# smallflyingpig/speech-to-image-translation-without-text

Measured on AMD Instinct MI355X. Metric: StackGAN-v2 3-stage G+D train-step images/sec at 256px, higher is better.
Workload: dtype f32

## Files before the change

include/s2i_hip.h:

```cpp
#ifndef S2I_HIP_H
#define S2I_HIP_H

#include <stddef.h>
#include <stdint.h>

#ifdef __cplusplus
extern "C" {
#endif

#define S2I_ABI_VERSION 4

#define S2I_CONV_K1      0
#define S2I_CONV_K3S1    1
#define S2I_CONV_K4S2    2
#define S2I_TCONV_K4S2   3

#define S2I_CONV_1D      4

#define S2I_ACT_NONE     0
#define S2I_ACT_GLU      1
#define S2I_ACT_LRELU    2
#define S2I_ACT_TANH     3
#define S2I_ACT_RELU     4

#define S2I_DT_F32       0
#define S2I_DT_BF16      1

#define S2I_PACK_PLAIN   0
#define S2I_PACK_UPFOLD  1

const char* s2i_last_error(void);
int  s2i_version(void);
int  s2i_set_tuning(const char* key, int value);
int  s2i_get_tuning(const char* key, int* value);
int  s2i_check_device(void);

typedef struct s2i_conv_desc {
  int kind;
  int B, H, W;
  int Cx;
  int Cc;
  int N;
  int wmode;
  int flip;
  int wR;
  int ldw;
  int act;
  int stats;
  int ldy;
  int groups;
  int nosplit;
  int kw, stride, pad;
  int tile_rows;
  int in_act;
  int in_groups;
} s2i_conv_desc;

size_t s2i_conv_workspace_bytes(const s2i_conv_desc* d);
int    s2i_conv_stat_parts(const s2i_conv_desc* d);
int s2i_conv_forward(const s2i_conv_desc* d, const float* x, const float* cvec, const float* w,
                     const float* bias, float* y, float* part, void* ws, size_t ws_bytes,
                     void* stream);

int s2i_conv_forward_cls(const s2i_conv_desc* d, const float* x, const float* cvec, const float* w,
                         const float* bias, const float* cls_bias, float* y, float* part, void* ws,
                         size_t ws_bytes, void* stream);

int s2i_conv_forward_in(const s2i_conv_desc* d, const float* x_raw, const float* in_coef, const float* w, float* y,
                        float* part, void* ws, size_t ws_bytes, void* stream);

int s2i_cvec_bias_table(const float* cvec, const float* packed, int B, int Cc, int Ip, int Op, int N,
                        float* table, void* ws , size_t ws_bytes, void* stream);
size_t s2i_border_sums_workspace_bytes(int B, int H, int W, int C);
int s2i_tap_sums(const float* dy, int B, int H, int W, int C, float* tapsum, void* ws, size_t ws_bytes,
                 void* stream);
int s2i_cvec_grads(const float* cvec, const float* packed, const float* tapsum, int B, int Cc, int Ip,
                   int Op, int N, int O, int I_total, float* dc, float* dw_oihw, int accumulate,
                   void* stream);

typedef struct s2i_wgrad_desc {
  int kind;
  int B, H, W;
  int Ca;
  int Cc;
  int N;
  int ldg;
  int swap;
  int fold;
  int O, I, KH, KW;
  int accumulate;
  int i_off;
  int I_total;
  int a_act;
  int a_groups;
} s2i_wgrad_desc;

size_t s2i_wgrad_workspace_bytes(const s2i_wgrad_desc* d);
int s2i_conv_wgrad(const s2i_wgrad_desc* d, const float* a, const float* cvec, const float* g,
                   float* grad_oihw, void* ws, size_t ws_bytes, void* stream);

int s2i_conv_wgrad_in_eligible(const s2i_wgrad_desc* d);
int s2i_conv_wgrad_in(const s2i_wgrad_desc* d, const float* a_raw, const float* a_coef, const float* g,
                      float* grad_oihw, void* ws, size_t ws_bytes, void* stream);


int s2i_conv_split_eligible(const s2i_conv_desc* d);
int s2i_conv_forward_split(const s2i_conv_desc* d, const float* x, const float* cvec,
                           const unsigned short* wsplit, int planes, int np, int kp, const float* bias,
                           const float* cls_bias, float* y, float* part, void* ws, size_t ws_bytes,
                           void* stream);
size_t s2i_wgrad_workspace_bytes_split(const s2i_wgrad_desc* d, int planes);
int s2i_conv_wgrad_split(const s2i_wgrad_desc* d, int planes, const float* a, const float* cvec,
                         const float* g, float* grad_oihw, void* ws, size_t ws_bytes, void* stream);
int s2i_split_packed_weight(const float* packed, int T, int R, int C, int planes, unsigned short* out_rc,
                            unsigned short* out_cr, void* stream);
// ... 243 lines not shown
```

speech_to_image_translation_without_text_amd/_lib.py:

```python
import ctypes
import os

import torch

_HERE = os.path.dirname(os.path.abspath(__file__))
LIB_PATH = os.path.join(_HERE, "libs2i_hip.so")

CONV_K1, CONV_K3S1, CONV_K4S2, TCONV_K4S2, CONV_1D = 0, 1, 2, 3, 4
ACT_NONE, ACT_GLU, ACT_LRELU, ACT_TANH, ACT_RELU = 0, 1, 2, 3, 4
PACK_PLAIN, PACK_UPFOLD = 0, 1
DT_F32, DT_BF16 = 0, 1
POOL_MAX3S2, POOL_AVG3S1, POOL_GLOBAL = 0, 1, 2
POOL_THEN_LRN, LRN_THEN_POOL = 0, 1
LOGMEL_BFT, LOGMEL_NHWC = 0, 1
ENC_LOSS_JEL, ENC_LOSS_L1, ENC_LOSS_DISTILL = 1, 2, 4
LOGMEL_TILE_FRAMES = 64
ABI_VERSION = 4

c_int, c_float, c_void_p, c_size_t, c_ll = (ctypes.c_int, ctypes.c_float, ctypes.c_void_p,
                                            ctypes.c_size_t, ctypes.c_longlong)


class ConvDesc(ctypes.Structure):
    _fields_ = [(n, c_int) for n in ("kind", "B", "H", "W", "Cx", "Cc", "N", "wmode", "flip", "wR",
                                     "ldw", "act", "stats", "ldy", "groups", "nosplit", "kw", "stride", "pad",
                                     "tile_rows", "in_act", "in_groups")]


class Conv2dDesc(ctypes.Structure):
    _fields_ = [(n, c_int) for n in ("B", "H", "W", "C", "ldx", "N", "kh", "kw", "sh", "sw", "ph", "pw", "Ho", "Wo",
                                     "ldy", "coff", "relu", "tile")]


class WgradDesc(ctypes.Structure):
    _fields_ = [(n, c_int) for n in ("kind", "B", "H", "W", "Ca", "Cc", "N", "ldg", "swap", "fold",
                                     "O", "I", "KH", "KW", "accumulate", "i_off", "I_total", "a_act", "a_groups")]


class PackItem(ctypes.Structure):
    _fields_ = [("w", c_void_p), ("packed", c_void_p)] + [(n, c_int) for n in ("O", "I", "KH", "KW", "Ip", "mode", "gx",
                                                                               "block0")]


class Pack16Item(ctypes.Structure):
    _fields_ = [("P", c_void_p), ("out", c_void_p)] + [(n, c_int) for n in (
        "R", "C", "kind", "flip", "transpose", "T", "nphase", "Nn", "Npad", "Kk", "CK", "gx", "gy", "block0")]


P = c_void_p
_SIGNATURES = {
    "s2i_last_error": (ctypes.c_char_p, []),
    "s2i_version": (c_int, []),
    "s2i_check_device": (c_int, []),
    "s2i_set_tuning": (c_int, [ctypes.c_char_p, c_int]),
    "s2i_get_tuning": (c_int, [ctypes.c_char_p, ctypes.POINTER(c_int)]),
    "s2i_conv_workspace_bytes": (c_size_t, [ctypes.POINTER(ConvDesc)]),
    "s2i_conv_stat_parts": (c_int, [ctypes.POINTER(ConvDesc)]),
    "s2i_conv_forward": (c_int, [ctypes.POINTER(ConvDesc), P, P, P, P, P, P, P, c_size_t, P]),
    "s2i_conv_forward_cls": (c_int, [ctypes.POINTER(ConvDesc), P, P, P, P, P, P, P, P, c_size_t, P]),
    "s2i_conv_forward_in": (c_int, [ctypes.POINTER(ConvDesc), P, P, P, P, P, P, c_size_t, P]),
    "s2i_conv_wgrad_in_eligible": (c_int, [ctypes.POINTER(WgradDesc)]),
    "s2i_conv_wgrad_in": (c_int, [ctypes.POINTER(WgradDesc), P, P, P, P, P, c_size_t, P]),
    "s2i_conv_split_eligible": (c_int, [ctypes.POINTER(ConvDesc)]),
    "s2i_conv_forward_split": (c_int, [ctypes.POINTER(ConvDesc), P, P, P, c_int, c_int, c_int, P, P, P, P, P, c_size_t, P]),
    "s2i_split_packed_weight": (c_int, [P, c_int, c_int, c_int, c_int, P, P, P]),
    "s2i_wgrad_workspace_bytes_split": (c_size_t, [ctypes.POINTER(WgradDesc), c_int]),
    "s2i_conv_wgrad_split": (c_int, [ctypes.POINTER(WgradDesc), c_int, P, P, P, P, P, c_size_t, P]),
    "s2i_conv_bf16_eligible": (c_int, [ctypes.POINTER(ConvDesc)]),
    "s2i_conv_bf16_workspace_bytes": (c_size_t, [ctypes.POINTER(ConvDesc)]),
    "s2i_conv_bf16_stat_parts": (c_int, [ctypes.POINTER(ConvDesc)]),
    "s2i_conv_bf16_weight_elems": (c_size_t, [ctypes.POINTER(ConvDesc)]),
    "s2i_conv_bf16_weight_layout": (c_int, [ctypes.POINTER(ConvDesc)]),
    "s2i_pack16_item_fill": (c_int, [ctypes.POINTER(ConvDesc), P, c_int, c_int, P, ctypes.POINTER(Pack16Item)]),
    "s2i_pack_conv_weights_bf16_batched": (c_int, [P, c_int, c_int, P]),
    "s2i_pack_conv_weight_bf16": (c_int, [ctypes.POINTER(ConvDesc), P, c_int, c_int, P, P]),
    "s2i_conv_forward_bf16": (c_int, [ctypes.POINTER(ConvDesc), P, P, P, P, P, P, c_size_t, P]),
    "s2i_conv_forward_dt": (c_int, [ctypes.POINTER(ConvDesc), P, c_int, P, P, P, P, P, c_int, P, P, c_size_t, P]),
    "s2i_wgrad_workspace_bytes_dt": (c_size_t, [ctypes.POINTER(WgradDesc), c_int, c_int]),
    "s2i_conv_wgrad_dt": (c_int, [ctypes.POINTER(WgradDesc), P, c_int, P, P, c_int, P, P, c_size_t, P]),
    "s2i_bn_act_forward_dt": (c_int, [c_int, P, c_ll, c_int, c_int, P, c_int, P, P, P]),
    "s2i_bn_act_bwd_reduce_dt": (c_int, [c_int, P, P, c_int, c_ll, c_int, c_int, P, c_int, P, c_int, P]),
    "s2i_bn_act_bwd_apply_dt": (c_int, [c_int, P, P, c_int, c_ll, c_int, c_int, P, P, c_int, P, P]),
    "s2i_act_backward_dt": (c_int, [c_int, P, P, c_int, c_ll, c_int, c_int, P, P]),
    "s2i_nchw_to_nhwc_dt": (c_int, [c_int, P, P, c_int, c_int, c_int, c_int, c_int, P]),
    "s2i_nhwc_to_nchw_dt": (c_int, [c_int, P, c_int, P, c_int, c_int, c_int, c_int, P]),
    "s2i_spatial_sum_dt": (c_int, [c_int, P, c_int, c_int, c_int, c_int, P, P, c_size_t, P]),
    "s2i_tap_sums_dt": (c_int, [c_int, P, c_int, c_int, c_int, c_int, P, P, c_size_t, P]),
    "s2i_cast": (c_int, [P, c_int, P, c_int, c_ll, P]),
    "s2i_cvec_bias_table": (c_int, [P, P, c_int, c_int, c_int, c_int, c_int, P, P, c_size_t, P]),
    "s2i_border_sums_workspace_bytes": (c_size_t, [c_int, c_int, c_int, c_int]),
    "s2i_tap_sums": (c_int, [P, c_int, c_int, c_int, c_int, P, P, c_size_t, P]),
    "s2i_cvec_grads": (c_int, [P, P, P, c_int, c_int, c_int, c_int, c_int, c_int, c_int, P, P, c_int, P]),
    "s2i_wgrad_workspace_bytes": (c_size_t, [ctypes.POINTER(WgradDesc)]),
    "s2i_conv_wgrad": (c_int, [ctypes.POINTER(WgradDesc), P, P, P, P, P, c_size_t, P]),
    "s2i_pack_conv_weight": (c_int, [P, P, c_int, c_int, c_int, c_int, c_int, c_int, P]),
    "s2i_pack_conv_weights_batched": (c_int, [P, c_int, c_int, c_int, P]),
    "s2i_bn_finalize": (c_int, [P, c_int, c_int, c_int, c_ll, P, P, P, P, P, c_float, c_float, P, P]),
    "s2i_bn_eval_coeffs": (c_int, [c_int, P, P, P, P, c_float, P, P]),
    "s2i_bn_act_forward": (c_int, [P, c_ll, c_int, c_int, P, c_int, P, P, P]),
    "s2i_colstats": (c_int, [P, c_ll, c_int, c_int, P, c_int, P]),
    "s2i_bn_act_bwd_reduce": (c_int, [P, P, c_int, c_ll, c_int, c_int, P, c_int, P, c_int, P]),
    "s2i_bn_bwd_finalize": (c_int, [P, c_int, c_int, c_int, c_ll, P, P, c_int, P, P]),
    "s2i_bn_act_bwd_apply": (c_int, [P, P, c_int, c_ll, c_int, c_int, P, P, c_int, P, P]),
    "s2i_act_backward": (c_int, [P, P, c_int, c_ll, c_int, c_int, P, P]),
    "s2i_glu_forward": (c_int, [P, c_ll, c_int, P, P]),
    "s2i_glu_backward": (c_int, [P, P, c_ll, c_int, P, P]),
    "s2i_nchw_to_nhwc": (c_int, [P, P, c_int, c_int, c_int, c_int, c_int, P]),
    "s2i_nhwc_to_nchw": (c_int, [P, c_int, P, c_int, c_int, c_int, c_int, P]),
# ... 152 lines not shown
```

speech_to_image_translation_without_text_amd/csrc/s2i_common.h:

```cpp
#pragma once
#include <hip/hip_runtime.h>
#include <stdio.h>
#include <stdarg.h>
#include "../../include/s2i_hip.h"

typedef float f32x16 __attribute__((ext_vector_type(16)));
typedef float f32x4 __attribute__((ext_vector_type(4)));

void s2i_set_error(const char* fmt, ...);

#define S2I_FAIL(...)            \
  do {                           \
    s2i_set_error(__VA_ARGS__);  \
    return 1;                    \
  } while (0)

#define S2I_REQUIRE(cond, ...)   \
  do {                           \
    if (!(cond)) S2I_FAIL(__VA_ARGS__); \
  } while (0)

#define S2I_LAUNCH_CHECK(name)                                          \
  do {                                                                  \
    hipError_t e__ = hipGetLastError();                                 \
    if (e__ != hipSuccess) S2I_FAIL("%s: launch failed: %s", name, hipGetErrorString(e__)); \
  } while (0)

static inline int s2i_ilog2(int v) {
  int l = 0;
  while ((1 << l) < v) ++l;
  return l;
}
static inline bool s2i_is_pow2(int v) { return v > 0 && (v & (v - 1)) == 0; }
static inline int s2i_cdiv(long long a, long long b) { return (int)((a + b - 1) / b); }

enum {
  S2I_TUNE_FWD_BM = 0,
  S2I_TUNE_FWD_MIN_CPS,
  S2I_TUNE_B16_V2,
  S2I_TUNE_B16_PERSIST,
  S2I_TUNE_FINALIZE_THREADS,
  S2I_TUNE_B16_DBG,
  S2I_TUNE_WGRAD16_BM,
  S2I_TUNE_WGRAD_BM,
  S2I_TUNE_COUNT
};
int s2i_tune(int key, int def);
```

speech_to_image_translation_without_text_amd/csrc/s2i_conv_fwd.hip:

```cpp
#include "s2i_igemm.h"

namespace {

template <int ASLOTS>
__device__ __forceinline__ void gather_rows(const IgemmP& p, int m0, int mrow, int kq, int s, int pad, int kw, int py, int px,
                                            int (&aoff)[ASLOTS], unsigned (&amask)[ASLOTS], int (&acoff)[ASLOTS]) {
#pragma unroll
  for (int i = 0; i < ASLOTS; ++i) {
    const int m = m0 + mrow + 32 * i;
    unsigned mask = 0;
    int base = 0, coff = 0;
    if (m < p.M) {
      int b, oy, ox;
      row_pixel(p, m, b, oy, ox);
      const int by = p.kind == S2I_CONV_1D ? oy : oy * s - pad, bx = ox * s - pad;
      mask = tap_mask(p.kind, kw, by, bx, p.H, p.W, py, px);
      base = (((b * p.H + by) * p.W + bx) * p.Cx + kq * 4) * 4;
      coff = (b * p.Cc + kq * 4) * 4;
    }
    aoff[i] = base;
    amask[i] = mask;
    acoff[i] = coff;
  }
}
// ... 541 lines not shown
    else if (act == S2I_ACT_TANH) v = tanhf(v);
    else if (act == S2I_ACT_RELU) v = fmaxf(v, 0.f);
    if (y16) reinterpret_cast<unsigned short*>(y)[row * ldy + n] = f2bf(v);
    else y[row * ldy + n] = v;
  }
}

__global__ __launch_bounds__(256) void splitk_reduce_stats_kernel(const float* __restrict__ slab, int S, long long rows,
                                                                  int N, float* __restrict__ y, int ldy,
                                                                  float* __restrict__ part, int nparts, int cpb,
                                                                  int ppg, long long Rg, int y16) {
  __shared__ f32x4 sh[2][256];
  const int tid = threadIdx.x;
  const int rpb = 256 / cpb;
  const int ql = tid % cpb, rl = tid / cpb;
  const int quad = blockIdx.y * cpb + ql;
  const int Q = N / 4;
  const int grp = blockIdx.x / ppg, pp = blockIdx.x - grp * ppg;
  const long long chunk = (Rg + ppg - 1) / ppg;
  const long long r0 = grp * Rg + pp * chunk;
  const long long gend = (grp + 1) * Rg < rows ? (grp + 1) * Rg : rows;
  const long long r1 = r0 + chunk < gend ? r0 + chunk : gend;
  const size_t sstride = (size_t)rows * N;
  f32x4 s0 = {0.f, 0.f, 0.f, 0.f}, s1 = {0.f, 0.f, 0.f, 0.f};
  if (quad < Q) {
    for (long long row = r0 + rl; row < r1; row += rpb) {
      const float* sp = slab + row * N + quad * 4;
      f32x4 v = *reinterpret_cast<const f32x4*>(sp);
      for (int s = 1; s < S; ++s) v += *reinterpret_cast<const f32x4*>(sp + s * sstride);
      if (y16) {
        unsigned short* yp = reinterpret_cast<unsigned short*>(y) + row * ldy + quad * 4;
        *reinterpret_cast<u32x2_t*>(yp) = u32x2_t{(unsigned)f2bf(v[0]) | ((unsigned)f2bf(v[1]) << 16),
                                                 (unsigned)f2bf(v[2]) | ((unsigned)f2bf(v[3]) << 16)};
      } else {
        *reinterpret_cast<f32x4*>(y + row * ldy + quad * 4) = v;
      }
      s0 += v;
      s1 += v * v;
    }
  }
  sh[0][tid] = s0;
  sh[1][tid] = s1;
  __syncthreads();
  if (rl == 0 && quad < Q) {
    for (int r = 1; r < rpb; ++r) {
      s0 += sh[0][r * cpb + ql];
      s1 += sh[1][r * cpb + ql];
    }
    *reinterpret_cast<f32x4*>(part + ((size_t)0 * nparts + blockIdx.x) * N + quad * 4) = s0;
    *reinterpret_cast<f32x4*>(part + ((size_t)1 * nparts + blockIdx.x) * N + quad * 4) = s1;
  }
}

template <int BM, int BN, int WM, int WN>
void launch_fwd(const IgemmP& p, dim3 grid, bool wt, bool ca32, hipStream_t st) {
  if (p.in_coef) {
    hipLaunchKernelGGL((igemm_fwd_kernel<BM, BN, WM, WN, false, true, true>), grid, dim3(256), 0, st, p);
    return;
  }
  if (wt) {
    if (ca32) hipLaunchKernelGGL((igemm_fwd_kernel<BM, BN, WM, WN, true, true>), grid, dim3(256), 0, st, p);
    else hipLaunchKernelGGL((igemm_fwd_kernel<BM, BN, WM, WN, true, false>), grid, dim3(256), 0, st, p);
  } else {
    if (ca32) hipLaunchKernelGGL((igemm_fwd_kernel<BM, BN, WM, WN, false, true>), grid, dim3(256), 0, st, p);
    else hipLaunchKernelGGL((igemm_fwd_kernel<BM, BN, WM, WN, false, false>), grid, dim3(256), 0, st, p);
  }
}

template <int BM, int BN, int WM, int WN>
static void launch_split(const IgemmP& p, dim3 grid, int planes, hipStream_t st) {
  if (planes == 1) hipLaunchKernelGGL((igemm_fwd_split_kernel<BM, BN, WM, WN, 1>), grid, dim3(256), 0, st, p);
  else if (planes == 2) hipLaunchKernelGGL((igemm_fwd_split_kernel<BM, BN, WM, WN, 2>), grid, dim3(256), 0, st, p);
  else hipLaunchKernelGGL((igemm_fwd_split_kernel<BM, BN, WM, WN, 3>), grid, dim3(256), 0, st, p);
}

}

int launch_igemm_fwd(const FwdPlan& pl, const IgemmP& p, dim3 grid, bool wt, bool ca32, hipStream_t st) {
  if (pl.bm == 96) launch_fwd<96, 128, 1, 4>(p, grid, wt, ca32, st);
  else if (pl.tile == 0) launch_fwd<128, 128, 2, 2>(p, grid, wt, ca32, st);
  else if (pl.tile == 1) launch_fwd<128, 64, 2, 2>(p, grid, wt, ca32, st);
  else launch_fwd<128, 32, 4, 1>(p, grid, wt, ca32, st);
  S2I_LAUNCH_CHECK("igemm_fwd");
  return 0;
}

int launch_igemm_fwd_split(const FwdPlan& pl, const IgemmP& p, dim3 grid, int planes, hipStream_t st) {
  if (pl.tile == 0) launch_split<128, 128, 2, 2>(p, grid, planes, st);
  else if (pl.tile == 1) launch_split<128, 64, 2, 2>(p, grid, planes, st);
  else launch_split<128, 32, 4, 1>(p, grid, planes, st);
  S2I_LAUNCH_CHECK("igemm_fwd_split");
  return 0;
}

int launch_small_n_conv(const s2i_conv_desc* d, const FwdPlan& pl, IgemmP p, hipStream_t st) {
  p.wt = d->wmode != 0;
  const int lpp = pl.Ca / 4, ppw = 64 / lpp;
  int sblocks = s2i_cdiv(pl.M, 4 * ppw);
  if (sblocks > 2048 / pl.nphases) sblocks = 2048 / pl.nphases;
  dim3 sgrid(sblocks, 1, pl.nphases);
  const size_t shb = (size_t)pl.T * pl.Ca * 4 * sizeof(float);
  if (lpp == 4) hipLaunchKernelGGL((small_n_conv_kernel<4>), sgrid, dim3(256), shb, st, p);
  else if (lpp == 8) hipLaunchKernelGGL((small_n_conv_kernel<8>), sgrid, dim3(256), shb, st, p);
  else hipLaunchKernelGGL((small_n_conv_kernel<16>), sgrid, dim3(256), shb, st, p);
  S2I_LAUNCH_CHECK("small_n_conv");
  return 0;
}

int launch_splitk_reduce(const s2i_conv_desc* d, const FwdPlan& pl, const float* bias, float* y, float* part, void* ws,
                         int y16, void* stream) {
  hipStream_t st = (hipStream_t)stream;
  if (d->stats && (d->N % 4) == 0 && (d->ldy % 4) == 0) {
    const int Q = d->N / 4;
    int cpb = 1;
    while (cpb < Q && cpb < 256) cpb <<= 1;
    const int groups = d->groups < 1 ? 1 : d->groups;
    const int nparts = stat_parts_for(pl, groups);
    hipLaunchKernelGGL(splitk_reduce_stats_kernel, dim3(nparts, (Q + cpb - 1) / cpb), dim3(256), 0, st,
                       (const float*)ws, pl.splitk, pl.Mrows, d->N, y, d->ldy, part, nparts, cpb, nparts / groups,
                       pl.Mrows / groups, y16);
    S2I_LAUNCH_CHECK("splitk_reduce_stats");
    return 0;
  }
  const long long total = pl.Mrows * d->N;
  int blocks = s2i_cdiv(total, 256);
  if (blocks > 4096) blocks = 4096;
  hipLaunchKernelGGL(splitk_reduce_kernel, dim3(blocks), dim3(256), 0, st, (const float*)ws, pl.splitk,
                     pl.Mrows, d->N, bias, d->act, y, d->ldy, y16);
  S2I_LAUNCH_CHECK("splitk_reduce");
  S2I_REQUIRE(!(d->stats && y16), "conv: bf16 output with statistics needs N %% 4 == 0 on a split-K layer");
  if (d->stats) return s2i_colstats(y, pl.Mrows, d->N, d->ldy, part, stat_parts_for(pl, 1), stream);
  return 0;
}

extern "C" int s2i_split_packed_weight(const float* packed, int T, int R, int C, int planes, unsigned short* out_rc,
                                       unsigned short* out_cr, void* stream) {
  S2I_REQUIRE(packed && (out_rc || out_cr) && T > 0 && R > 0 && C > 0 && planes >= 1 && planes <= 3,
              "split_packed_weight: bad args");
  dim3 grid(s2i_cdiv(C, 32), s2i_cdiv(R, 32), T);
  hipLaunchKernelGGL(split_packed_kernel, grid, dim3(256), 0, (hipStream_t)stream, packed, out_rc, out_cr, R, C, planes,
                     (long long)T * R * C);
  S2I_LAUNCH_CHECK("split_packed_weight");
  return 0;
}
```

speech_to_image_translation_without_text_amd/csrc/s2i_runtime.hip:

```cpp
#include "s2i_common.h"
#include <string.h>

static thread_local char g_err[512] = "";

void s2i_set_error(const char* fmt, ...) {
  va_list ap;
  va_start(ap, fmt);
  vsnprintf(g_err, sizeof(g_err), fmt, ap);
  va_end(ap);
}

extern "C" const char* s2i_last_error(void) { return g_err; }

extern "C" int s2i_version(void) { return S2I_ABI_VERSION; }

extern "C" int s2i_check_device(void) {
  int dev = 0;
  hipError_t e = hipGetDevice(&dev);
  if (e != hipSuccess) S2I_FAIL("check_device: hipGetDevice: %s", hipGetErrorString(e));
  hipDeviceProp_t prop;
  e = hipGetDeviceProperties(&prop, dev);
  if (e != hipSuccess) S2I_FAIL("check_device: hipGetDeviceProperties: %s", hipGetErrorString(e));
  if (strncmp(prop.gcnArchName, "gfx950", 6) != 0)
    S2I_FAIL("check_device: kernels are built for gfx950 only, device %d is %s", dev, prop.gcnArchName);
  return 0;
}

#include <stdlib.h>
static const char* const g_tune_names[S2I_TUNE_COUNT] = {"fwd_bm", "fwd_min_cps", "b16_v2", "b16_persist", "finalize_threads", "b16_dbg",
                                                            "wgrad16_bm", "wgrad_bm"};
static int g_tune_val[S2I_TUNE_COUNT];
static bool g_tune_set[S2I_TUNE_COUNT];

static int tune_index(const char* key, size_t len) {
  for (int i = 0; i < S2I_TUNE_COUNT; ++i)
    if (strlen(g_tune_names[i]) == len && strncmp(g_tune_names[i], key, len) == 0) return i;
  return -1;
}

namespace {
struct TuneInit {
  TuneInit() {
    const char* e = getenv("S2I_TUNE");
    while (e && *e) {
      const char* eq = strchr(e, '=');
      if (!eq) break;
      const int i = tune_index(e, (size_t)(eq - e));
      if (i >= 0) { g_tune_val[i] = atoi(eq + 1); g_tune_set[i] = true; }
      const char* c = strchr(eq, ',');
      e = c ? c + 1 : nullptr;
    }
  }
} g_tune_init;
}

int s2i_tune(int key, int def) { return g_tune_set[key] ? g_tune_val[key] : def; }

extern "C" int s2i_set_tuning(const char* key, int value) {
  const int i = key ? tune_index(key, strlen(key)) : -1;
  if (i < 0) S2I_FAIL("set_tuning: unknown key '%s'", key ? key : "(null)");
  g_tune_val[i] = value;
  g_tune_set[i] = value >= 0;
  return 0;
}

extern "C" int s2i_get_tuning(const char* key, int* value) {
  const int i = key ? tune_index(key, strlen(key)) : -1;
  if (i < 0 || !value) S2I_FAIL("get_tuning: unknown key '%s'", key ? key : "(null)");
  *value = g_tune_set[i] ? g_tune_val[i] : -1;
  return 0;
}
```

speech_to_image_translation_without_text_amd/csrc/s2i_wgrad.hip:

```cpp
#include "s2i_igemm.h"

namespace {

struct WgradP {
  const float* __restrict__ a;
  const float* __restrict__ cvec;
  const float* __restrict__ g;
  float* __restrict__ slab;
  int B, H, W, Ca, Cc, Cin;
  int Ho, Wo, lgWo, lgHoWo;
  int M, N, ldg, K, T, kind;
  int cps, nchunks;
  int a16, g16;
  unsigned a_bytes, c_bytes, g_bytes;
  const float* __restrict__ a_coef;
  int a_groups, a_ipg;
};

__device__ __forceinline__ bool wgrad_col(const WgradP& p, int kcol, int kw, int& c, int& dy, int& dx) {
  c = 0;
  dy = 0;
  dx = 0;
  if (kcol >= p.K) return false;
  const int t = kcol / p.Cin;
// ... 556 lines not shown
  float* outp = p.slab + (size_t)blockIdx.x * p.K * 4;
  for (int e = tid; e < 9 * LPP * 4; e += 256) {
    const f32x4 v = red[0][e] + red[1][e] + red[2][e] + red[3][e];
    *reinterpret_cast<f32x4*>(outp + (size_t)e * 4) = v;
  }
}

__global__ __launch_bounds__(256) void slab_sum_tree_kernel(float* __restrict__ slab, int S, int n4) {
  __shared__ f32x4 sh[256];
  const int tid = threadIdx.x;
  const int e = blockIdx.x * 4 + (tid & 3), sl = tid >> 2;
  f32x4 v = {0.f, 0.f, 0.f, 0.f};
  if (e < n4)
    for (int s = sl; s < S; s += 64) v += *reinterpret_cast<const f32x4*>(slab + ((size_t)s * n4 + e) * 4);
  sh[tid] = v;
  __syncthreads();
  for (int h = 32; h >= 1; h >>= 1) {
    if (sl < h) sh[tid] += sh[tid + h * 4];
    __syncthreads();
  }
  if (sl == 0 && e < n4) *reinterpret_cast<f32x4*>(slab + (size_t)e * 4) = sh[tid];
}

__global__ __launch_bounds__(256) void slab_sum_kernel(float* __restrict__ slab, int S, long long n4) {
  for (long long e = (long long)blockIdx.x * blockDim.x + threadIdx.x; e < n4;
       e += (long long)gridDim.x * blockDim.x) {
    f32x4 v = *reinterpret_cast<const f32x4*>(slab + e * 4);
    for (int s = 1; s < S; ++s) v += *reinterpret_cast<const f32x4*>(slab + ((size_t)s * n4 + e) * 4);
    *reinterpret_cast<f32x4*>(slab + e * 4) = v;
  }
}

__global__ __launch_bounds__(256) void wgrad_finish_kernel(const float* __restrict__ slab, int S, int K, int N,
                                                           int Cg, int O, int I, int Tp, int T, int swap, int fold,
                                                           int accumulate, int RT, float* __restrict__ grad,
                                                           int i_off, int I_total) {
  extern __shared__ float tile[];
  const int tid = threadIdx.x;
  const int ncols = swap ? I : O, nrows = swap ? O : I;
  const int c0 = blockIdx.x * 32, r0 = blockIdx.y * RT;
  const size_t sstride = (size_t)K * N;
  const int nload = T * RT * 32;
  for (int e = tid; e < nload; e += 256) {
    const int c_l = e & 31;
    const int r_l = (e >> 5) % RT;
    const int t = (e >> 5) / RT;
    const int c = c0 + c_l, r = r0 + r_l;
    float v = 0.f;
    if (c < ncols && r < nrows) {
      const float* sp = slab + ((size_t)t * Cg + r) * N + c;
      for (int s = 0; s < S; ++s) v += sp[s * sstride];
    }
    tile[(t * RT + r_l) * 33 + c_l] = v;
  }
  __syncthreads();
  const int nout = 32 * RT * Tp;
  for (int w = tid; w < nout; w += 256) {
    const int tapo = w % Tp;
    const int rest = w / Tp;
    int o_l, i_l, r_l, c_l;
    if (swap) { i_l = rest & 31; o_l = rest >> 5; r_l = o_l; c_l = i_l; }
    else { i_l = rest % RT; o_l = rest / RT; r_l = i_l; c_l = o_l; }
    const int o = swap ? r0 + o_l : c0 + o_l;
    const int i = swap ? c0 + i_l : r0 + i_l;
    if (o >= O || i >= I) continue;
    float v;
    if (fold) {
      const int ky = tapo / 3, kx = tapo - ky * 3;
      v = 0.f;
#pragma unroll
      for (int ay = 0; ay < 2; ++ay)
#pragma unroll
        for (int ax = 0; ax < 2; ++ax) {
          const int t = ((2 - ky) + ay) * 4 + (2 - kx) + ax;
          v += tile[(t * RT + r_l) * 33 + c_l];
        }
    } else {
      v = tile[(tapo * RT + r_l) * 33 + c_l];
    }
    float* gp = grad + ((size_t)o * I_total + i_off + i) * Tp + tapo;
    *gp = accumulate ? *gp + v : v;
  }
}

}

template <int BM, int BN, int WM, int WN>
static void launch_wgrad_split(const WgradP& p, dim3 grid, int planes, hipStream_t st) {
  if (planes == 1) hipLaunchKernelGGL((igemm_wgrad_split_kernel<BM, BN, WM, WN, 1>), grid, dim3(256), 0, st, p);
  else if (planes == 2) hipLaunchKernelGGL((igemm_wgrad_split_kernel<BM, BN, WM, WN, 2>), grid, dim3(256), 0, st, p);
  else hipLaunchKernelGGL((igemm_wgrad_split_kernel<BM, BN, WM, WN, 3>), grid, dim3(256), 0, st, p);
}

static int conv_wgrad_impl(const s2i_wgrad_desc* d, int planes, const float* a, const float* cvec, const float* g,
                           float* grad_oihw, void* ws, size_t ws_bytes, void* stream, int a16 = 0, int g16 = 0, const float* a_coef = nullptr) {
  WgPlan pl;
  if (plan_wgrad(d, &pl, (a16 && g16) ? 16 : ((planes || a16 || g16) ? 1 : 0))) return 1;
  S2I_REQUIRE(!(planes && (a16 || g16)), "wgrad(split): bf16 tensors go through s2i_conv_wgrad_dt");
  S2I_REQUIRE(!(pl.small_n && g16), "wgrad: the <= 4 channel gradient stream expects an fp32 output gradient");
  S2I_REQUIRE((a || d->Ca == 0) && g && grad_oihw, "wgrad: null operand");
  S2I_REQUIRE(d->Cc == 0 || cvec != nullptr, "wgrad: cvec is null but Cc > 0");
  const size_t need = (size_t)pl.splitk * pl.K * d->N * sizeof(float);
  S2I_REQUIRE(ws && ws_bytes >= need, "wgrad: workspace too small (%zu < %zu)", ws_bytes, need);
  hipStream_t st = (hipStream_t)stream;
  WgradP p;
  p.a = a; p.cvec = cvec; p.g = g; p.slab = (float*)ws;
// ... 22 lines not shown
    q.nchunks = s2i_cdiv(pl.M, 64);
    q.cps = s2i_cdiv(q.nchunks, pl.splitk);
    dim3 g32(1, 1, s2i_cdiv(q.nchunks, q.cps));
    pl.splitk = (int)g32.z;
    pl.gridK = 1; pl.gridN = 1;
    hipLaunchKernelGGL((igemm_wgrad_b16_kernel<64, 64, 2, 2, true>), g32, dim3(256), 0, st, q);
  } else if (a16 && g16 && !pl.small_n && d->Cc == 0 && (pl.Cin % 8) == 0 && (d->N % 8) == 0 && (d->ldg % 8) == 0) {
    WgradP q = p;
    q.nchunks = s2i_cdiv(pl.M, 64);
    q.cps = s2i_cdiv(q.nchunks, pl.splitk);
    dim3 g16grid(pl.gridK, pl.gridN, s2i_cdiv(q.nchunks, q.cps));
    S2I_REQUIRE((int)g16grid.z <= pl.splitk, "wgrad(bf16): split plan mismatch");
    pl.splitk = (int)g16grid.z;
    if (pl.tile == 7) hipLaunchKernelGGL((igemm_wgrad_b16_kernel<256, 256, 4, 4>), g16grid, dim3(1024), 0, st, q);
    else if (pl.tile == 6) hipLaunchKernelGGL((igemm_wgrad_b16_kernel<256, 128, 4, 2>), g16grid, dim3(512), 0, st, q);
    else if (pl.tile == 0) hipLaunchKernelGGL((igemm_wgrad_b16_kernel<128, 128, 2, 2>), g16grid, dim3(256), 0, st, q);
    else if (pl.tile == 1) hipLaunchKernelGGL((igemm_wgrad_b16_kernel<128, 64, 2, 2>), g16grid, dim3(256), 0, st, q);
    else if (pl.tile == 2) hipLaunchKernelGGL((igemm_wgrad_b16_kernel<128, 32, 4, 1>), g16grid, dim3(256), 0, st, q);
    else hipLaunchKernelGGL((igemm_wgrad_b16_kernel<64, 64, 2, 2>), g16grid, dim3(256), 0, st, q);
  } else if (pl.rows3) {
    dim3 g3(d->Ca == 32 ? 1 : 3, pl.gridN, pl.splitk);
    if (d->Ca == 32 && pl.bn3 == 64) hipLaunchKernelGGL((wgrad_k3_rows_kernel<32, 64, 3, 1, 3>), g3, dim3(192), 0, st, p);
    else if (d->Ca == 32) hipLaunchKernelGGL((wgrad_k3_rows_kernel<32, 32, 3, 1, 3>), g3, dim3(192), 0, st, p);
    else if (pl.bn3 == 128) hipLaunchKernelGGL((wgrad_k3_rows_kernel<64, 128, 2, 2, 1>), g3, dim3(256), 0, st, p);
    else if (pl.bn3 == 64) hipLaunchKernelGGL((wgrad_k3_rows_kernel<64, 64, 2, 2, 1>), g3, dim3(256), 0, st, p);
    else hipLaunchKernelGGL((wgrad_k3_rows_kernel<64, 32, 2, 1, 1>), g3, dim3(128), 0, st, p);
  } else if (planes && !pl.small_n) {
    if (pl.tile == 0) launch_wgrad_split<128, 128, 2, 2>(p, grid, planes, st);
    else if (pl.tile == 1) launch_wgrad_split<128, 64, 2, 2>(p, grid, planes, st);
    else if (pl.tile == 2) launch_wgrad_split<128, 32, 4, 1>(p, grid, planes, st);
    else launch_wgrad_split<64, 64, 2, 2>(p, grid, planes, st);
  } else if (pl.small_n) {
    if (d->Ca == 16) hipLaunchKernelGGL(small_n_wgrad_kernel<4>, dim3(pl.splitk), dim3(256), 0, st, p);
    else if (d->Ca == 32) hipLaunchKernelGGL(small_n_wgrad_kernel<8>, dim3(pl.splitk), dim3(256), 0, st, p);
    else hipLaunchKernelGGL(small_n_wgrad_kernel<16>, dim3(pl.splitk), dim3(256), 0, st, p);
  } else if (pl.tile == 9) hipLaunchKernelGGL((igemm_wgrad_kernel<256, 256, 4, 4>), grid, dim3(1024), 0, st, p);
  else if (pl.tile == 8) hipLaunchKernelGGL((igemm_wgrad_kernel<256, 128, 4, 2>), grid, dim3(512), 0, st, p);
  else if (pl.tile == 0 && a_coef) hipLaunchKernelGGL((igemm_wgrad_kernel<128, 128, 2, 2, true>), grid, dim3(256), 0, st, p);
  else if (pl.tile == 0) hipLaunchKernelGGL((igemm_wgrad_kernel<128, 128, 2, 2>), grid, dim3(256), 0, st, p);
  else if (pl.tile == 1) hipLaunchKernelGGL((igemm_wgrad_kernel<128, 64, 2, 2>), grid, dim3(256), 0, st, p);
  else if (pl.tile == 2) hipLaunchKernelGGL((igemm_wgrad_kernel<128, 32, 4, 1>), grid, dim3(256), 0, st, p);
  else if (pl.tile == 3) hipLaunchKernelGGL((igemm_wgrad_kernel<64, 64, 2, 2>), grid, dim3(256), 0, st, p);
  else if (pl.tile == 4) hipLaunchKernelGGL((igemm_wgrad_kernel<96, 64, 3, 1>), grid, dim3(192), 0, st, p);
  else hipLaunchKernelGGL((igemm_wgrad_kernel<96, 32, 3, 1>), grid, dim3(192), 0, st, p);
  S2I_LAUNCH_CHECK("igemm_wgrad");
  {
    const int ncols = d->swap ? d->I : d->O, nrows = d->swap ? d->O : d->I;
    int RT = 8;
    while (RT > 1 && (long long)s2i_cdiv(ncols, 32) * s2i_cdiv(nrows, RT) < 128) RT >>= 1;
    dim3 fgrid(s2i_cdiv(ncols, 32), s2i_cdiv(nrows, RT));
    const size_t shb = (size_t)pl.T * RT * 33 * sizeof(float);
    int S = pl.splitk;
    const long long kn = (long long)pl.K * d->N;
    if (pl.small_n || (S >= 32 && (kn % 4) == 0 && kn / 4 < (1 << 18))) {
      hipLaunchKernelGGL(slab_sum_tree_kernel, dim3(s2i_cdiv(kn / 4, 4)), dim3(256), 0, st, (float*)ws, S, (int)(kn / 4));
      S2I_LAUNCH_CHECK("slab_sum_tree");
      S = 1;
    } else if (S > 2 && (kn % 4) == 0) {
      int sb = s2i_cdiv(kn / 4, 256);
      if (sb > 4096) sb = 4096;
      hipLaunchKernelGGL(slab_sum_kernel, dim3(sb), dim3(256), 0, st, (float*)ws, S, kn / 4);
      S2I_LAUNCH_CHECK("slab_sum");
      S = 1;
    }
    hipLaunchKernelGGL(wgrad_finish_kernel, fgrid, dim3(256), shb, st, (const float*)ws, S, pl.K, d->N,
                       pl.Cin, d->O, d->I, d->KH * d->KW, pl.T, d->swap, d->fold, d->accumulate, RT, grad_oihw,
                       d->i_off, d->I_total > 0 ? d->I_total : d->I);
  }
  S2I_LAUNCH_CHECK("wgrad_finish");
  return 0;
}

extern "C" int s2i_conv_wgrad_in(const s2i_wgrad_desc* d, const float* a_raw, const float* a_coef, const float* g,
                                 float* grad_oihw, void* ws, size_t ws_bytes, void* stream) {
  S2I_REQUIRE(a_coef != nullptr, "wgrad(apply-on-load): null coefficient table");
  return conv_wgrad_impl(d, 0, a_raw, nullptr, g, grad_oihw, ws, ws_bytes, stream, 0, 0, a_coef);
}

extern "C" int s2i_conv_wgrad_dt(const s2i_wgrad_desc* d, const void* a, int a_dtype, const float* cvec, const void* g,
                                 int g_dtype, float* grad_oihw, void* ws, size_t ws_bytes, void* stream) {
  S2I_REQUIRE((a_dtype == S2I_DT_F32 || a_dtype == S2I_DT_BF16) && (g_dtype == S2I_DT_F32 || g_dtype == S2I_DT_BF16),
              "wgrad: unknown dtype");
  return conv_wgrad_impl(d, 0, (const float*)a, cvec, (const float*)g, grad_oihw, ws, ws_bytes, stream,
                         a_dtype == S2I_DT_BF16, g_dtype == S2I_DT_BF16);
}

extern "C" int s2i_conv_wgrad(const s2i_wgrad_desc* d, const float* a, const float* cvec, const float* g,
                              float* grad_oihw, void* ws, size_t ws_bytes, void* stream) {
  return conv_wgrad_impl(d, 0, a, cvec, g, grad_oihw, ws, ws_bytes, stream);
}

extern "C" int s2i_conv_wgrad_split(const s2i_wgrad_desc* d, int planes, const float* a, const float* cvec,
                                    const float* g, float* grad_oihw, void* ws, size_t ws_bytes, void* stream) {
  S2I_REQUIRE(planes >= 1 && planes <= 3, "wgrad(split): need 1 to 3 bf16 planes");
  return conv_wgrad_impl(d, planes, a, cvec, g, grad_oihw, ws, ws_bytes, stream);
}
```

Before: 783.1.

## Vectorize split-K reduction, row-parallel stats reduce, and wide wgrad finish kernels

Adds float4-vectorized variants of the split-K reduction paths: a grid-stride vector reduce with fused bias/activation, a stats kernel that assigns several rows per block and reduces partial sums through shared memory, a wide slab-sum, and a wide wgrad finish kernel that loads four columns per thread with batched slab loads. All are gated by a new reduce_v2 tuning knob that defaults on, with fallbacks to the old kernels. The aim is fewer memory transactions and more loads in flight across split-K slabs. It also adds a public splitk_reduce entry point and atomic launch counters for each reduction form, which add a small host cost per launch.

After: 788.8 (median of 6 runs). No clear change (+0.7%).

```diff
diff --git a/include/s2i_hip.h b/include/s2i_hip.h
--- a/include/s2i_hip.h
+++ b/include/s2i_hip.h
@@ -34,6 +34,7 @@
 int  s2i_set_tuning(const char* key, int value);
 int  s2i_get_tuning(const char* key, int* value);
 int  s2i_check_device(void);
+long long s2i_reduction_launches(int form);
 
 typedef struct s2i_conv_desc {
   int kind;
@@ -61,6 +62,9 @@
 int s2i_conv_forward(const s2i_conv_desc* d, const float* x, const float* cvec, const float* w,
                      const float* bias, float* y, float* part, void* ws, size_t ws_bytes,
                      void* stream);
+
+int s2i_splitk_reduce(const float* slabs, int S, long long rows, int N, int groups, int nparts, const float* bias,
+                      int act, void* y, int y_dtype, int ldy, float* part, void* stream);
 
 int s2i_conv_forward_cls(const s2i_conv_desc* d, const float* x, const float* cvec, const float* w,
                          const float* bias, const float* cls_bias, float* y, float* part, void* ws,
diff --git a/speech_to_image_translation_without_text_amd/_lib.py b/speech_to_image_translation_without_text_amd/_lib.py
--- a/speech_to_image_translation_without_text_amd/_lib.py
+++ b/speech_to_image_translation_without_text_amd/_lib.py
@@ -54,6 +54,8 @@
     "s2i_check_device": (c_int, []),
     "s2i_set_tuning": (c_int, [ctypes.c_char_p, c_int]),
     "s2i_get_tuning": (c_int, [ctypes.c_char_p, ctypes.POINTER(c_int)]),
+    "s2i_reduction_launches": (c_ll, [c_int]),
+    "s2i_splitk_reduce": (c_int, [P, c_int, c_ll, c_int, c_int, c_int, P, c_int, P, c_int, c_int, P, P]),
     "s2i_conv_workspace_bytes": (c_size_t, [ctypes.POINTER(ConvDesc)]),
     "s2i_conv_stat_parts": (c_int, [ctypes.POINTER(ConvDesc)]),
     "s2i_conv_forward": (c_int, [ctypes.POINTER(ConvDesc), P, P, P, P, P, P, P, c_size_t, P]),
diff --git a/speech_to_image_translation_without_text_amd/csrc/s2i_common.h b/speech_to_image_translation_without_text_amd/csrc/s2i_common.h
--- a/speech_to_image_translation_without_text_amd/csrc/s2i_common.h
+++ b/speech_to_image_translation_without_text_amd/csrc/s2i_common.h
@@ -43,6 +43,21 @@
   S2I_TUNE_B16_DBG,
   S2I_TUNE_WGRAD16_BM,
   S2I_TUNE_WGRAD_BM,
+  S2I_TUNE_REDUCE_V2,
   S2I_TUNE_COUNT
 };
 int s2i_tune(int key, int def);
+
+enum {
+  S2I_RED_STATS_V1 = 0,
+  S2I_RED_STATS_ROWS,
+  S2I_RED_PLAIN_V1,
+  S2I_RED_PLAIN_VEC,
+  S2I_RED_FINISH_V1,
+  S2I_RED_FINISH_WIDE,
+  S2I_RED_SLABSUM_V1,
+  S2I_RED_SLABSUM_WIDE,
+  S2I_RED_TREE,
+  S2I_RED_COUNT
+};
+void s2i_note_reduction(int form);
diff --git a/speech_to_image_translation_without_text_amd/csrc/s2i_conv_fwd.hip b/speech_to_image_translation_without_text_amd/csrc/s2i_conv_fwd.hip
--- a/speech_to_image_translation_without_text_amd/csrc/s2i_conv_fwd.hip
+++ b/speech_to_image_translation_without_text_amd/csrc/s2i_conv_fwd.hip
@@ -617,6 +617,100 @@
   }
 }
 
+__global__ __launch_bounds__(256) void splitk_reduce_vec_kernel(const float* __restrict__ slab, int S, long long rows, int N,
+                                                                const float* __restrict__ bias, int act,
+                                                                float* __restrict__ y, int ldy, int y16) {
+  const int Q = N / 4;
+  const long long total4 = rows * Q;
+  const size_t sstride = (size_t)rows * N;
+  for (long long e = (long long)blockIdx.x * blockDim.x + threadIdx.x; e < total4;
+       e += (long long)gridDim.x * blockDim.x) {
+    const long long row = e / Q;
+    const int quad = (int)(e - row * Q);
+    const float* sp = slab + e * 4;
+    f32x4 v = {0.f, 0.f, 0.f, 0.f};
+    for (int s0 = 0; s0 < S; s0 += 8) {
+      f32x4 t[8];
+#pragma unroll
+      for (int j = 0; j < 8; ++j)
+        if (s0 + j < S) t[j] = *reinterpret_cast<const f32x4*>(sp + (size_t)(s0 + j) * sstride);
+#pragma unroll
+      for (int j = 0; j < 8; ++j)
+        if (s0 + j < S) v += t[j];
+    }
+    if (bias) v += *reinterpret_cast<const f32x4*>(bias + quad * 4);
+#pragma unroll
+    for (int n = 0; n < 4; ++n) {
+      if (act == S2I_ACT_LRELU) v[n] = v[n] > 0.f ? v[n] : 0.2f * v[n];
+      else if (act == S2I_ACT_TANH) v[n] = tanhf(v[n]);
+      else if (act == S2I_ACT_RELU) v[n] = fmaxf(v[n], 0.f);
+    }
+    if (y16) {
+      unsigned short* yp = reinterpret_cast<unsigned short*>(y) + row * ldy + quad * 4;
+      *reinterpret_cast<u32x2_t*>(yp) = u32x2_t{(unsigned)f2bf(v[0]) | ((unsigned)f2bf(v[1]) << 16),
+                                               (unsigned)f2bf(v[2]) | ((unsigned)f2bf(v[3]) << 16)};
+    } else {
+      *reinterpret_cast<f32x4*>(y + row * ldy + quad * 4) = v;
+    }
+  }
+}
+
+__global__ __launch_bounds__(256) __attribute__((amdgpu_waves_per_eu(8, 8))) void splitk_reduce_stats_rows_kernel(const float* __restrict__ slab, int S, long long rows,
+                                                                       int N, float* __restrict__ y, int ldy,
+                                                                       float* __restrict__ part, int nparts, int cpb,
+                                                                       int ppg, long long Rg, int y16, int prpb) {
+  __shared__ f32x4 sh[256];
+  const int tid = threadIdx.x;
+  const int ql = tid % cpb, rl = tid / cpb;
+  const int quad = blockIdx.y * cpb + ql;
+  const int Q = N / 4;
+  const int grp = blockIdx.x / ppg, pp = blockIdx.x - grp * ppg;
+  const long long chunk = (Rg + ppg - 1) / ppg;
+  const long long r0 = grp * Rg + pp * chunk;
+  const long long gend = (grp + 1) * Rg < rows ? (grp + 1) * Rg : rows;
+  const long long r1 = r0 + chunk < gend ? r0 + chunk : gend;
+  const size_t sstride = (size_t)rows * N;
+  const long long row = r0 + rl;
+  f32x4 v = {0.f, 0.f, 0.f, 0.f};
+  if (quad < Q && row < r1) {
+    const float* sp = slab + row * N + quad * 4;
+    for (int s0 = 0; s0 < S; s0 += 8) {
+      f32x4 t[8];
+#pragma unroll
+      for (int j = 0; j < 8; ++j)
+        if (s0 + j < S) t[j] = *reinterpret_cast<const f32x4*>(sp + (size_t)(s0 + j) * sstride);
+#pragma unroll
+      for (int j = 0; j < 8; ++j)
+        if (s0 + j < S) v = (s0 + j == 0) ? t[j] : v + t[j];
+    }
+    if (y16) {
+      unsigned short* yp = reinterpret_cast<unsigned short*>(y) + row * ldy + quad * 4;
+      *reinterpret_cast<u32x2_t*>(yp) = u32x2_t{(unsigned)f2bf(v[0]) | ((unsigned)f2bf(v[1]) << 16),
+                                               (unsigned)f2bf(v[2]) | ((unsigned)f2bf(v[3]) << 16)};
+    } else {
+      *reinterpret_cast<f32x4*>(y + row * ldy + quad * 4) = v;
+    }
+  }
+  sh[tid] = v;
+  __syncthreads();
+  if (rl == 0 && quad < Q) {
+    const int n = r1 > r0 ? (int)(r1 - r0) : 0;
+    f32x4 s0 = {0.f, 0.f, 0.f, 0.f}, s1 = {0.f, 0.f, 0.f, 0.f};
+    for (int l = 0; l < prpb && l < n; ++l) {
+      f32x4 a0 = {0.f, 0.f, 0.f, 0.f}, a1 = {0.f, 0.f, 0.f, 0.f};
+      for (int i = l; i < n; i += prpb) {
+        const f32x4 w = sh[i * cpb + ql];
+        a0 += w;
+        a1 += w * w;
+      }
+      if (l == 0) { s0 = a0; s1 = a1; }
+      else { s0 += a0; s1 += a1; }
+    }
+    *reinterpret_cast<f32x4*>(part + ((size_t)0 * nparts + blockIdx.x) * N + quad * 4) = s0;
+    *reinterpret_cast<f32x4*>(part + ((size_t)1 * nparts + blockIdx.x) * N + quad * 4) = s1;
+  }
+}
+
 template <int BM, int BN, int WM, int WN>
 void launch_fwd(const IgemmP& p, dim3 grid, bool wt, bool ca32, hipStream_t st) {
   if (p.in_coef) {
@@ -672,30 +766,74 @@
   return 0;
 }
 
+static int splitk_reduce_launch(const float* ws, int S, long long rows, int N, int groups, int nparts, int stats,
+                                const float* bias, int act, float* y, int ldy, int y16, float* part, hipStream_t st) {
+  const bool v2 = s2i_tune(S2I_TUNE_REDUCE_V2, 1) != 0;
+  const bool vec_ok = (N % 4) == 0 && (ldy % 4) == 0;
+  if (stats && vec_ok) {
+    const int Q = N / 4;
+    int cpb = 1;
+    while (cpb < Q && cpb < 256) cpb <<= 1;
+    const int ppg = nparts / groups;
+    const long long Rg = rows / groups;
+    const long long chunk = (Rg + ppg - 1) / ppg;
+    int cpr = cpb < 64 ? cpb : 64;
+    while (cpr > 1 && 256 / cpr < chunk) cpr >>= 1;
+    if (v2 && 256 / cpr >= chunk && (cpr >= 8 || cpr == cpb)) {
+      hipLaunchKernelGGL(splitk_reduce_stats_rows_kernel, dim3(nparts, (Q + cpr - 1) / cpr), dim3(256), 0, st, ws, S, rows,
+                         N, y, ldy, part, nparts, cpr, ppg, Rg, y16, 256 / cpb);
+      s2i_note_reduction(S2I_RED_STATS_ROWS);
+    } else {
+      hipLaunchKernelGGL(splitk_reduce_stats_kernel, dim3(nparts, (Q + cpb - 1) / cpb), dim3(256), 0, st, ws, S, rows, N, y,
+                         ldy, part, nparts, cpb, ppg, Rg, y16);
+      s2i_note_reduction(S2I_RED_STATS_V1);
+    }
+    S2I_LAUNCH_CHECK("splitk_reduce_stats");
+    return 0;
+  }
+  const long long total = rows * N;
+  if (v2 && vec_ok && ((uintptr_t)y & (y16 ? 7u : 15u)) == 0 && (!bias || ((uintptr_t)bias & 15u) == 0)) {
+    int blocks = s2i_cdiv(total / 4, 256);
+    if (blocks > 8192) blocks = 8192;
+    hipLaunchKernelGGL(splitk_reduce_vec_kernel, dim3(blocks), dim3(256), 0, st, ws, S, rows, N, bias, act, y, ldy, y16);
+    s2i_note_reduction(S2I_RED_PLAIN_VEC);
+  } else {
+    int blocks = s2i_cdiv(total, 256);
+    if (blocks > 4096) blocks = 4096;
+    hipLaunchKernelGGL(splitk_reduce_kernel, dim3(blocks), dim3(256), 0, st, ws, S, rows, N, bias, act, y, ldy, y16);
+    s2i_note_reduction(S2I_RED_PLAIN_V1);
+  }
+  S2I_LAUNCH_CHECK("splitk_reduce");
+  return 0;
+}
+
 int launch_splitk_reduce(const s2i_conv_desc* d, const FwdPlan& pl, const float* bias, float* y, float* part, void* ws,
                          int y16, void* stream) {
   hipStream_t st = (hipStream_t)stream;
-  if (d->stats && (d->N % 4) == 0 && (d->ldy % 4) == 0) {
-    const int Q = d->N / 4;
-    int cpb = 1;
-    while (cpb < Q && cpb < 256) cpb <<= 1;
-    const int groups = d->groups < 1 ? 1 : d->groups;
-    const int nparts = stat_parts_for(pl, groups);
-    hipLaunchKernelGGL(splitk_reduce_stats_kernel, dim3(nparts, (Q + cpb - 1) / cpb), dim3(256), 0, st,
-                       (const float*)ws, pl.splitk, pl.Mrows, d->N, y, d->ldy, part, nparts, cpb, nparts / groups,
-                       pl.Mrows / groups, y16);
-    S2I_LAUNCH_CHECK("splitk_reduce_stats");
-    return 0;
-  }
-  const long long total = pl.Mrows * d->N;
-  int blocks = s2i_cdiv(total, 256);
-  if (blocks > 4096) blocks = 4096;
-  hipLaunchKernelGGL(splitk_reduce_kernel, dim3(blocks), dim3(256), 0, st, (const float*)ws, pl.splitk,
-                     pl.Mrows, d->N, bias, d->act, y, d->ldy, y16);
-  S2I_LAUNCH_CHECK("splitk_reduce");
+  const bool fused = d->stats && (d->N % 4) == 0 && (d->ldy % 4) == 0;
+  const int groups = d->groups < 1 ? 1 : d->groups;
+  if (splitk_reduce_launch((const float*)ws, pl.splitk, pl.Mrows, d->N, groups, fused ? stat_parts_for(pl, groups) : 0,
+                           fused, bias, d->act, y, d->ldy, y16, part, st))
+    return 1;
+  if (fused) return 0;
   S2I_REQUIRE(!(d->stats && y16), "conv: bf16 output with statistics needs N %% 4 == 0 on a split-K layer");
   if (d->stats) return s2i_colstats(y, pl.Mrows, d->N, d->ldy, part, stat_parts_for(pl, 1), stream);
   return 0;
+}
+
+extern "C" int s2i_splitk_reduce(const float* slabs, int S, long long rows, int N, int groups, int nparts, const float* bias,
+                                 int act, void* y, int y_dtype, int ldy, float* part, void* stream) {
+  S2I_REQUIRE(slabs && y && S >= 1 && rows > 0 && N > 0 && ldy >= N, "splitk_reduce: bad args");
+  S2I_REQUIRE(y_dtype == S2I_DT_F32 || y_dtype == S2I_DT_BF16, "splitk_reduce: unknown dtype");
+  if (groups < 1) groups = 1;
+  if (part) {
+    S2I_REQUIRE((N % 4) == 0 && (ldy % 4) == 0, "splitk_reduce: statistics need N %% 4 == 0 and ldy %% 4 == 0");
+    S2I_REQUIRE(!bias && act == S2I_ACT_NONE, "splitk_reduce: statistics are taken of the plain sum (no bias, no activation)");
+    S2I_REQUIRE(nparts >= groups && (nparts % groups) == 0 && (rows % groups) == 0,
+                "splitk_reduce: %d partials / %lld rows do not split into %d groups", nparts, rows, groups);
+  }
+  return splitk_reduce_launch(slabs, S, rows, N, groups, nparts, part != nullptr, bias, act, (float*)y, ldy,
+                              y_dtype == S2I_DT_BF16, part, (hipStream_t)stream);
 }
 
 extern "C" int s2i_split_packed_weight(const float* packed, int T, int R, int C, int planes, unsigned short* out_rc,
diff --git a/speech_to_image_translation_without_text_amd/csrc/s2i_runtime.hip b/speech_to_image_translation_without_text_amd/csrc/s2i_runtime.hip
--- a/speech_to_image_translation_without_text_amd/csrc/s2i_runtime.hip
+++ b/speech_to_image_translation_without_text_amd/csrc/s2i_runtime.hip
@@ -28,7 +28,7 @@
 
 #include <stdlib.h>
 static const char* const g_tune_names[S2I_TUNE_COUNT] = {"fwd_bm", "fwd_min_cps", "b16_v2", "b16_persist", "finalize_threads", "b16_dbg",
-                                                            "wgrad16_bm", "wgrad_bm"};
+                                                            "wgrad16_bm", "wgrad_bm", "reduce_v2"};
 static int g_tune_val[S2I_TUNE_COUNT];
 static bool g_tune_set[S2I_TUNE_COUNT];
 
@@ -70,3 +70,13 @@
   *value = g_tune_set[i] ? g_tune_val[i] : -1;
   return 0;
 }
+
+#include <atomic>
+static std::atomic<long long> g_red_launches[S2I_RED_COUNT];
+
+void s2i_note_reduction(int form) { g_red_launches[form].fetch_add(1, std::memory_order_relaxed); }
+
+extern "C" long long s2i_reduction_launches(int form) {
+  if (form < 0 || form >= S2I_RED_COUNT) return -1;
+  return g_red_launches[form].load(std::memory_order_relaxed);
+}
diff --git a/speech_to_image_translation_without_text_amd/csrc/s2i_wgrad.hip b/speech_to_image_translation_without_text_amd/csrc/s2i_wgrad.hip
--- a/speech_to_image_translation_without_text_amd/csrc/s2i_wgrad.hip
+++ b/speech_to_image_translation_without_text_amd/csrc/s2i_wgrad.hip
@@ -632,6 +632,97 @@
       for (int s = 0; s < S; ++s) v += sp[s * sstride];
     }
     tile[(t * RT + r_l) * 33 + c_l] = v;
+  }
+  __syncthreads();
+  const int nout = 32 * RT * Tp;
+  for (int w = tid; w < nout; w += 256) {
+    const int tapo = w % Tp;
+    const int rest = w / Tp;
+    int o_l, i_l, r_l, c_l;
+    if (swap) { i_l = rest & 31; o_l = rest >> 5; r_l = o_l; c_l = i_l; }
+    else { i_l = rest % RT; o_l = rest / RT; r_l = i_l; c_l = o_l; }
+    const int o = swap ? r0 + o_l : c0 + o_l;
+    const int i = swap ? c0 + i_l : r0 + i_l;
+    if (o >= O || i >= I) continue;
+    float v;
+    if (fold) {
+      const int ky = tapo / 3, kx = tapo - ky * 3;
+      v = 0.f;
+#pragma unroll
+      for (int ay = 0; ay < 2; ++ay)
+#pragma unroll
+        for (int ax = 0; ax < 2; ++ax) {
+          const int t = ((2 - ky) + ay) * 4 + (2 - kx) + ax;
+          v += tile[(t * RT + r_l) * 33 + c_l];
+        }
+    } else {
+      v = tile[(tapo * RT + r_l) * 33 + c_l];
+    }
+    float* gp = grad + ((size_t)o * I_total + i_off + i) * Tp + tapo;
+    *gp = accumulate ? *gp + v : v;
+  }
+}
+
+__global__ __launch_bounds__(256) void slab_sum_wide_kernel(float* __restrict__ slab, int S, long long n4) {
+  for (long long e = (long long)blockIdx.x * blockDim.x + threadIdx.x; e < n4;
+       e += (long long)gridDim.x * blockDim.x) {
+    const float* sp = slab + e * 4;
+    f32x4 v = {0.f, 0.f, 0.f, 0.f};
+    for (int s0 = 0; s0 < S; s0 += 8) {
+      f32x4 t[8];
+#pragma unroll
+      for (int j = 0; j < 8; ++j)
+        if (s0 + j < S) t[j] = *reinterpret_cast<const f32x4*>(sp + (size_t)(s0 + j) * n4 * 4);
+#pragma unroll
+      for (int j = 0; j < 8; ++j)
+        if (s0 + j < S) v = (s0 + j == 0) ? t[j] : v + t[j];
+    }
+    *reinterpret_cast<f32x4*>(slab + e * 4) = v;
+  }
+}
+
+__global__ __launch_bounds__(256) void wgrad_finish_wide_kernel(const float* __restrict__ slab, int S, int K, int N,
+                                                                int Cg, int O, int I, int Tp, int T, int swap, int fold,
+                                                                int accumulate, int RT, float* __restrict__ grad,
+                                                                int i_off, int I_total) {
+  extern __shared__ float tile[];
+  const int tid = threadIdx.x;
+  const int ncols = swap ? I : O, nrows = swap ? O : I;
+  const int c0 = blockIdx.x * 32, r0 = blockIdx.y * RT;
+  const size_t sstride = (size_t)K * N;
+  const int nload4 = T * RT * 8;
+  for (int e0 = tid; e0 < nload4; e0 += 4 * 256) {
+    f32x4 v[4];
+    const float* sp[4];
+#pragma unroll
+    for (int k = 0; k < 4; ++k) {
+      const int e = e0 + k * 256;
+      const int c = c0 + (e & 7) * 4, r = r0 + (e >> 3) % RT, t = (e >> 3) / RT;
+      v[k] = f32x4{0.f, 0.f, 0.f, 0.f};
+      sp[k] = (e < nload4 && c < ncols && r < nrows) ? slab + ((size_t)t * Cg + r) * N + c : nullptr;
+    }
+    for (int s0 = 0; s0 < S; s0 += 2) {
+      f32x4 a[4], b[4];
+#pragma unroll
+      for (int k = 0; k < 4; ++k) {
+        if (sp[k]) a[k] = *reinterpret_cast<const f32x4*>(sp[k] + (size_t)s0 * sstride);
+        if (sp[k] && s0 + 1 < S) b[k] = *reinterpret_cast<const f32x4*>(sp[k] + (size_t)(s0 + 1) * sstride);
+      }
+#pragma unroll
+      for (int k = 0; k < 4; ++k) {
+        if (sp[k]) v[k] += a[k];
+        if (sp[k] && s0 + 1 < S) v[k] += b[k];
+      }
+    }
+#pragma unroll
+    for (int k = 0; k < 4; ++k) {
+      const int e = e0 + k * 256;
+      if (e >= nload4) continue;
+      const int c_l = (e & 7) * 4, r_l = (e >> 3) % RT, t = (e >> 3) / RT;
+      float* tp = tile + (t * RT + r_l) * 33 + c_l;
+#pragma unroll
+      for (int j = 0; j < 4; ++j) tp[j] = c0 + c_l + j < ncols ? v[k][j] : 0.f;
+    }
   }
   __syncthreads();
   const int nout = 32 * RT * Tp;
@@ -760,20 +851,31 @@
     const size_t shb = (size_t)pl.T * RT * 33 * sizeof(float);
     int S = pl.splitk;
     const long long kn = (long long)pl.K * d->N;
+    const int v2 = s2i_tune(S2I_TUNE_REDUCE_V2, 1);
+    const bool wide = v2 != 0 && (d->N % 4) == 0;
     if (pl.small_n || (S >= 32 && (kn % 4) == 0 && kn / 4 < (1 << 18))) {
       hipLaunchKernelGGL(slab_sum_tree_kernel, dim3(s2i_cdiv(kn / 4, 4)), dim3(256), 0, st, (float*)ws, S, (int)(kn / 4));
       S2I_LAUNCH_CHECK("slab_sum_tree");
+      s2i_note_reduction(S2I_RED_TREE);
       S = 1;
-    } else if (S > 2 && (kn % 4) == 0) {
+    } else if (S > 2 && (kn % 4) == 0 && !(wide && (v2 & 2))) {
       int sb = s2i_cdiv(kn / 4, 256);
       if (sb > 4096) sb = 4096;
-      hipLaunchKernelGGL(slab_sum_kernel, dim3(sb), dim3(256), 0, st, (float*)ws, S, kn / 4);
+      if (v2) hipLaunchKernelGGL(slab_sum_wide_kernel, dim3(sb), dim3(256), 0, st, (float*)ws, S, kn / 4);
+      else hipLaunchKernelGGL(slab_sum_kernel, dim3(sb), dim3(256), 0, st, (float*)ws, S, kn / 4);
       S2I_LAUNCH_CHECK("slab_sum");
+      s2i_note_reduction(v2 ? S2I_RED_SLABSUM_WIDE : S2I_RED_SLABSUM_V1);
       S = 1;
     }
-    hipLaunchKernelGGL(wgrad_finish_kernel, fgrid, dim3(256), shb, st, (const float*)ws, S, pl.K, d->N,
-                       pl.Cin, d->O, d->I, d->KH * d->KW, pl.T, d->swap, d->fold, d->accumulate, RT, grad_oihw,
-                       d->i_off, d->I_total > 0 ? d->I_total : d->I);
+    if (wide)
+      hipLaunchKernelGGL(wgrad_finish_wide_kernel, fgrid, dim3(256), shb, st, (const float*)ws, S, pl.K, d->N,
+                         pl.Cin, d->O, d->I, d->KH * d->KW, pl.T, d->swap, d->fold, d->accumulate, RT, grad_oihw,
+                         d->i_off, d->I_total > 0 ? d->I_total : d->I);
+    else
+      hipLaunchKernelGGL(wgrad_finish_kernel, fgrid, dim3(256), shb, st, (const float*)ws, S, pl.K, d->N,
+                         pl.Cin, d->O, d->I, d->KH * d->KW, pl.T, d->swap, d->fold, d->accumulate, RT, grad_oihw,
+                         d->i_off, d->I_total > 0 ? d->I_total : d->I);
+    s2i_note_reduction(wide ? S2I_RED_FINISH_WIDE : S2I_RED_FINISH_V1);
   }
   S2I_LAUNCH_CHECK("wgrad_finish");
   return 0;
```
